# wahn/rs_pbrt

Measured on NVIDIA B200. Metric: Mrays/s, higher is better.
Workload: dtype f32

## Files before the change

### rs_pbrt_b200/csrc/pb_kernels.cuh

```cuda
#pragma once
#include "pb_bsdf.cuh"
#include "pb_interaction.cuh"
#include "pb_sobol.cuh"
#include "pb_texture.cuh"
#include "pb_material.cuh"

namespace pb {

#define PB_TRACE_THREADS 128
#define PB_TRACE_SMEM_BYTES 49152
#define PB_SHADE_THREADS 128
#define PB_SMEM_SOBOL_BYTES 49152

#ifdef PB_HOST_EMU
PB_D void mbar_init(uint64_t*, uint32_t) {}
PB_D void mbar_fence_init() {}
PB_D void mbar_expect_tx(uint64_t*, uint32_t) {}
PB_D void tma_bulk_g2s(void* dst_smem, const void* src_gmem, uint32_t bytes, uint64_t*) { memcpy(dst_smem, src_gmem, bytes); }
PB_D void mbar_wait(uint64_t*, uint32_t) { __syncthreads(); }
#define PB_DYNAMIC_SMEM(name) unsigned char* name = emu::g_dyn_smem
#else
#define PB_DYNAMIC_SMEM(name) extern __shared__ __align__(16) unsigned char name[]
PB_D void mbar_fence_init() { asm volatile("fence.mbarrier_init.release.cluster;" ::: "memory"); }
PB_D uint32_t smem_u32(const void* p) { return (uint32_t)__cvta_generic_to_shared(p); }
// ... 267 lines not shown
    const uint2 a = tris[3 * (size_t)i], b = tris[3 * (size_t)i + 1], c = tris[3 * (size_t)i + 2];
    const uint32_t v0 = a.x, v1 = a.y, v2 = b.x, mesh = b.y, material = c.x;
    const int area_light = (int)c.y;
    uint32_t err = 0;
    if (mesh == 0xffffffffu) {
        if (v0 >= n_instances) err = 5;
        else {
            tv[3 * (size_t)i] = make_float4(__uint_as_float(v0), 0.0f, 0.0f, 0.0f);
            tv[3 * (size_t)i + 1] = make_float4(0.0f, 0.0f, 0.0f, 0.0f);
            tv[3 * (size_t)i + 2] = make_float4(0.0f, __uint_as_float(0xffffffffu), __uint_as_float(0xffffffffu), __uint_as_float((uint32_t)TRI_INSTANCE));
            tidx[i] = make_uint4(0, 0, 0, 0);
        }
    } else if (mesh >= n_meshes) err = 1;
    else {
        const DMeshRec m = meshes[mesh];
        if (v0 >= m.n_verts || v1 >= m.n_verts || v2 >= m.n_verts) err = 2;
        else if (material != 0xffffffffu && material >= n_materials) err = 3;
        else if (area_light >= (int)n_lights) err = 4;
        else if (area_light >= 0 && (m.flags & (TRI_ALPHA | TRI_SHADOW_ALPHA))) err = 6;
        else {
            if (material == 0xffffffffu) status[1] = 1u;
            const float* p0 = vp + 3 * (size_t)(m.vbase + v0);
            const float* p1 = vp + 3 * (size_t)(m.vbase + v1);
            const float* p2 = vp + 3 * (size_t)(m.vbase + v2);
            tv[3 * (size_t)i] = make_float4(p0[0], p0[1], p0[2], p1[0]);
            tv[3 * (size_t)i + 1] = make_float4(p1[1], p1[2], p2[0], p2[1]);
            tv[3 * (size_t)i + 2] = make_float4(p2[2], __uint_as_float(material), __uint_as_float((uint32_t)area_light), __uint_as_float(m.flags));
            tidx[i] = make_uint4(m.vbase + v0, m.vbase + v1, m.vbase + v2, mesh);
        }
    }
    if (err) atomicMax(status, err);
}

__global__ void __launch_bounds__(256) k_wide_build(const float4* __restrict__ nodes, uint32_t n_nodes, float4* __restrict__ wide) {
    const uint32_t i = blockIdx.x * blockDim.x + threadIdx.x;
    if (i >= n_nodes) return;
    const float4 m1 = nodes[2 * (size_t)i + 1];
    const uint32_t meta = __float_as_uint(m1.w);
    if (meta & 0xffffu) return;
    const uint32_t c[2] = {i + 1u, __float_as_uint(m1.z)};
    float4 a[2], b[2];
    uint32_t ref[2];
    for (int k = 0; k < 2; ++k) {
        a[k] = nodes[2 * (size_t)c[k]];
        b[k] = nodes[2 * (size_t)c[k] + 1];
        const uint32_t cm = __float_as_uint(b[k].w), np = cm & 0xffffu;
        ref[k] = np ? (__float_as_uint(b[k].z) | (np << PB_WIDE_LEAF_SHIFT)) : c[k];
    }
    float4* o = wide + 4 * (size_t)i;
    o[0] = make_float4(a[0].x, a[0].y, a[0].z, a[0].w);
    o[1] = make_float4(b[0].x, b[0].y, a[1].x, a[1].y);
    o[2] = make_float4(a[1].z, a[1].w, b[1].x, b[1].y);
    o[3] = make_float4(__uint_as_float(ref[0]), __uint_as_float(ref[1]), __uint_as_float((meta >> 16) & 3u), 0.0f);
}
#ifndef PB_WIDE_MIN_BLOCKS
#define PB_WIDE_MIN_BLOCKS 0
#endif
#ifndef PB_WIDE_INST_MIN_BLOCKS
#define PB_WIDE_INST_MIN_BLOCKS 8
#endif
#if PB_WIDE_MIN_BLOCKS > 0
#define PB_WIDE_BOUNDS __launch_bounds__(PB_TRACE_THREADS, PB_WIDE_MIN_BLOCKS)
#else
#define PB_WIDE_BOUNDS __launch_bounds__(PB_TRACE_THREADS)
#endif
__global__ void PB_WIDE_BOUNDS k_trace_wide_plain(DScene sc, TraceIO io, const uint32_t* __restrict__ d_nrays, uint32_t* __restrict__ cursor, DCounters* cnt, int walk_steps) {
    trace_rays_wide<false>(sc, sc.wide, sc.tri_verts, io, *d_nrays, cursor, cnt, walk_steps);
}
__global__ void __launch_bounds__(PB_TRACE_THREADS, PB_WIDE_INST_MIN_BLOCKS) k_trace_wide_inst(DScene sc, TraceIO io, const uint32_t* __restrict__ d_nrays, uint32_t* __restrict__ cursor,
                                                                                             DCounters* cnt, int walk_steps) {
    trace_rays_wide<true>(sc, sc.wide, sc.tri_verts, io, *d_nrays, cursor, cnt, walk_steps);
}

__global__ void PB_WIDE_BOUNDS k_trace_wide_spec(DScene sc, TraceIO io, const uint32_t* __restrict__ d_nrays,
                                                                                        uint32_t* __restrict__ cursor, DCounters* cnt, int walk_steps) {
    trace_rays_wide_spec(sc, sc.wide, sc.tri_verts, io, *d_nrays, cursor, cnt, walk_steps);
}

__global__ void __launch_bounds__(256) k_rayprep(const float4* __restrict__ rays, const uint32_t* __restrict__ d_nrays, float4* __restrict__ pre) {
    const uint32_t n = *d_nrays;
    for (uint32_t i = blockIdx.x * blockDim.x + threadIdx.x; i < n; i += gridDim.x * blockDim.x) {
        const float4 a = rays[2 * (size_t)i], b = rays[2 * (size_t)i + 1];
        const RayPre r = make_ray(mk3(a.x, a.y, a.z), mk3(b.x, b.y, b.z));
        float4 p0, p1;
        pack_ray(r, p0, p1);
        pre[2 * (size_t)i] = p0;
        pre[2 * (size_t)i + 1] = p1;
    }
}

__global__ void __launch_bounds__(256) k_sort(DScene sc, DPaths ps, DLightGrid grid, uint32_t spatial, uint32_t instancing, const uint32_t* __restrict__ queue,
                                             const uint32_t* __restrict__ d_count, uint32_t* __restrict__ cls_queue, uint32_t cls_stride,
                                             uint32_t* __restrict__ cls_count, uint32_t* __restrict__ reset_count_out, uint32_t* __restrict__ reset_nrays) {
    if (blockIdx.x == 0 && threadIdx.x == 0) { *reset_count_out = 0u; *reset_nrays = 0u; }
    const uint32_t count = *d_count;
    const uint32_t lane = threadIdx.x & 31;
    const uint32_t total = (count + 31u) & ~31u;
    for (uint32_t qi = blockIdx.x * blockDim.x + threadIdx.x; qi < total; qi += gridDim.x * blockDim.x) {
        uint32_t cls = 0xffffffffu, slot = 0;
        if (qi < count) {
            slot = queue[qi];
            cls = 0;
            if (__float_as_uint(ps.L[slot].w) & PF_HAS_RAY) {
                float4 h = ps.hit[slot];
                int prim = __float_as_int(h.x);
                if (prim >= 0) {
                    float4 c = __ldg(sc.tri_verts + 3 * (size_t)prim + 2);
                    uint32_t mat = __float_as_uint(c.y);
                    const uint32_t inst = sc.n_instances ? ps.hit_inst[slot] : 0xffffffffu;
// ... 745 lines not shown
```

### rs_pbrt_b200/csrc/pb_trace.cuh

```cuda
#pragma once
#include "pb_scene.cuh"

namespace pb {

struct RayPre {
    V3 o, d;
    V3 inv_dir;
    int neg[3];
    uint32_t negmask;
    int kx, ky, kz;
    float sx, sy, sz;
};

PB_D RayPre make_ray(V3 o, V3 d) {
    RayPre r;
    r.o = o;
    r.d = d;
    r.inv_dir = mk3(1.0f / d.x, 1.0f / d.y, 1.0f / d.z);
    r.neg[0] = r.inv_dir.x < 0.0f;
    r.neg[1] = r.inv_dir.y < 0.0f;
    r.neg[2] = r.inv_dir.z < 0.0f;
    r.negmask = (uint32_t)r.neg[0] | ((uint32_t)r.neg[1] << 1) | ((uint32_t)r.neg[2] << 2);
    r.kz = maxdim(abs3(d));
    r.kx = r.kz + 1; if (r.kx == 3) r.kx = 0;
// ... 625 lines not shown
            }
            if (!entered) {
                leaf_n = 0;
                if (!done) {
                    uint32_t nxt = 0;
                    PB_WPOP();
                    PB_WGOTO();
                }
            }
        }
        if (active && done) {
            if (INST && !any_hit && !hit_flag) best_prim = -1;
            const uint32_t slot = dest & PB_RAY_SLOT_MASK, kind = dest >> 30;
            if (kind == RAY_SHADOW) io.occl[slot] = best_prim >= 0 ? 1u : 0u;
            else {
                const float4 rec = make_float4(__int_as_float(best_prim), best.b0, best.b1, best.b2);
                if (kind == RAY_EXTEND) { io.hit[slot] = rec; if (INST) io.hit_inst[slot] = (uint32_t)best_inst; }
                else { io.mis_hit[slot] = rec; if (INST) io.mis_inst[slot] = (uint32_t)best_inst; }
            }
            active = false;
        }
    }
#undef PB_WPOP
#undef PB_WGOTO
#undef PB_WPUSH
    uint32_t a = n_closest, b = n_shadow;
    for (int o = 16; o > 0; o >>= 1) { a += __shfl_xor_sync(FULL, a, o); b += __shfl_xor_sync(FULL, b, o); }
    if (lane == 0) {
        if (a) atomicAdd(&cnt->closest_rays, (unsigned long long)a);
        if (b) atomicAdd(&cnt->shadow_rays, (unsigned long long)b);
    }
}

PB_D void trace_rays_wide_spec(const DScene& sc, const float4* __restrict__ wide, const float4* __restrict__ tris, const TraceIO& io, uint32_t n_rays,
                               uint32_t* __restrict__ cursor, DCounters* cnt, int walk_steps) {
    const unsigned FULL = 0xffffffffu;
    const int lane = threadIdx.x & 31;
    constexpr int NS = PB_WIDE_STACK_ENTRIES;
    __shared__ uint32_t s_ref[NS][PB_TRACE_THREADS_];
    __shared__ float s_tmin[NS][PB_TRACE_THREADS_];
    uint32_t l_ref[64 - NS];
    float l_tmin[64 - NS];
    RayPre r;
    float t_max = 0.0f, cur_tmin = 0.0f, leaf2_tmin = 0.0f;
    THit best;
    int best_prim = -1;
    uint32_t sp = 0, cur = 0, dest = 0, leaf1 = 0, leaf2 = 0;
    bool active = false, any_hit = false, exhausted = n_rays == 0, have_cur = false;
    uint32_t n_closest = 0, n_shadow = 0;
    const float neg_inf = __int_as_float((int)0xff800000);
#define PB_SPOP()                                                                                               \
    do {                                                                                                        \
        found = false;                                                                                          \
        while (sp != 0u) {                                                                                      \
            --sp;                                                                                               \
            const uint32_t e_ = sp < (uint32_t)NS ? s_ref[sp][threadIdx.x] : l_ref[sp - NS];                    \
            const float m_ = sp < (uint32_t)NS ? s_tmin[sp][threadIdx.x] : l_tmin[sp - NS];                     \
            if (m_ < t_max) { nxt = e_; tm = m_; found = true; break; }                                         \
        }                                                                                                       \
    } while (0)
#define PB_SROUTE()                                                                                             \
    do {                                                                                                        \
        for (;;) {                                                                                              \
            if (!found) { have_cur = false; break; }                                                            \
            if (!(nxt >> PB_WIDE_LEAF_SHIFT)) { cur = nxt; cur_tmin = tm; have_cur = true; break; }             \
            if (!leaf1) { leaf1 = nxt; PB_SPOP(); continue; }                                                   \
            leaf2 = nxt; leaf2_tmin = tm; have_cur = false; break;                                              \
        }                                                                                                       \
    } while (0)
    for (;;) {
        unsigned idle = __ballot_sync(FULL, !active);
        bool done = false;
        if (idle && !exhausted) {
            uint32_t base = 0;
            if (lane == 0) base = atomicAdd(cursor, (uint32_t)__popc(idle));
            base = __shfl_sync(FULL, base, 0);
            if (base >= n_rays) exhausted = true;
            const uint32_t my = base + (uint32_t)__popc(idle & ((1u << lane) - 1u));
            if (!active && my < n_rays) {
                const uint32_t qi = io.perm ? __ldg(io.perm + my) : my;
                const float4 a = ldg4_stream(io.rays + 2 * (size_t)qi), b = ldg4_stream(io.rays + 2 * (size_t)qi + 1);
                t_max = a.w;
                dest = __float_as_uint(b.w);
                any_hit = (dest >> 30) == RAY_SHADOW;
                r = make_ray(mk3(a.x, a.y, a.z), mk3(b.x, b.y, b.z));
                best_prim = -1;
                best.t = 0.0f; best.b0 = best.b1 = best.b2 = 0.0f;
                sp = 0; cur = 0; cur_tmin = neg_inf; leaf1 = 0; leaf2 = 0;
                active = true;
                if (any_hit) n_shadow++; else n_closest++;
                const float4 n0 = ldg4_keep(sc.nodes), n1 = ldg4_keep(sc.nodes + 1);
                have_cur = slab_test(n0, n1, r, t_max);
            }
        }
        if (!__any_sync(FULL, active)) break;
        for (int step = 0; step < walk_steps; ++step) {
            if (!(active && have_cur)) break;
            const float4* rec = wide + 4 * (size_t)cur;
            const float4 f0 = ldg4_keep(rec), f1 = ldg4_keep(rec + 1), f2 = ldg4_keep(rec + 2), f3 = ldg4_keep(rec + 3);
            float tm0, tm1;
            const bool h0 = slab_geo(f0.x, f0.y, f0.z, f0.w, f1.x, f1.y, r, tm0) && tm0 < t_max;
            const bool h1 = slab_geo(f1.z, f1.w, f2.x, f2.y, f2.z, f2.w, r, tm1) && tm1 < t_max;
            const bool neg = ((r.negmask >> (__float_as_uint(f3.z) & 3u)) & 1u) != 0u;
            const uint32_t ref0 = __float_as_uint(f3.x), ref1 = __float_as_uint(f3.y);
            const uint32_t ref_n = neg ? ref1 : ref0, ref_f = neg ? ref0 : ref1;
            const bool hn = neg ? h1 : h0, hf = neg ? h0 : h1;
            const float tn = neg ? tm1 : tm0, tf = neg ? tm0 : tm1;
            if (hn && hf) {
                if (sp < (uint32_t)NS) { s_ref[sp][threadIdx.x] = ref_f; s_tmin[sp][threadIdx.x] = tf; }
                else { l_ref[sp - NS] = ref_f; l_tmin[sp - NS] = tf; }
                ++sp;
            }
            uint32_t nxt = hn ? ref_n : ref_f;
            float tm = hn ? tn : tf;
            bool found = hn || hf;
            if (!found) PB_SPOP();
            PB_SROUTE();
        }
        if (active && leaf1) {
            const uint32_t leaf_n = leaf1 >> PB_WIDE_LEAF_SHIFT, leaf_off = leaf1 & ((1u << PB_WIDE_LEAF_SHIFT) - 1u);
            for (uint32_t i = 0; i < leaf_n; ++i) {
                const float4* tp = tris + 3 * (size_t)(leaf_off + i);
                const float4 a = ldg4_stream(tp), b = ldg4_stream(tp + 1), c = ldg4_stream(tp + 2);
                THit h;
                if (tri_test(mk3(a.x, a.y, a.z), mk3(a.w, b.x, b.y), mk3(b.z, b.w, c.x), r, t_max, h)) {
                    t_max = h.t;
                    best = h;
                    best_prim = (int)(leaf_off + i);
                    if (any_hit) { done = true; break; }
                }
            }
            leaf1 = 0;
            if (!done) {
                bool resume = false;
                if (leaf2) {
                    if (leaf2_tmin < t_max) leaf1 = leaf2;
                    leaf2 = 0;
                    resume = true;
                } else if (have_cur && !(cur_tmin < t_max)) { have_cur = false; resume = true; }
                if (resume) {
                    uint32_t nxt = 0;
                    float tm = 0.0f;
                    bool found;
                    PB_SPOP();
                    PB_SROUTE();
                }
            }
        }
        if (active && !done && !leaf1 && !leaf2 && !have_cur) done = true;
        if (active && done) {
            const uint32_t slot = dest & PB_RAY_SLOT_MASK, kind = dest >> 30;
            if (kind == RAY_SHADOW) io.occl[slot] = best_prim >= 0 ? 1u : 0u;
            else {
                const float4 rec = make_float4(__int_as_float(best_prim), best.b0, best.b1, best.b2);
                if (kind == RAY_EXTEND) io.hit[slot] = rec; else io.mis_hit[slot] = rec;
            }
            active = false;
        }
    }
#undef PB_SPOP
#undef PB_SROUTE
    uint32_t a = n_closest, b = n_shadow;
    for (int o = 16; o > 0; o >>= 1) { a += __shfl_xor_sync(FULL, a, o); b += __shfl_xor_sync(FULL, b, o); }
    if (lane == 0) {
        if (a) atomicAdd(&cnt->closest_rays, (unsigned long long)a);
        if (b) atomicAdd(&cnt->shadow_rays, (unsigned long long)b);
    }
}

}
```

### rs_pbrt_b200/csrc/pbrt_gpu.cu

```cuda
#include <sched.h>

#include <algorithm>
#include <chrono>
#include <cmath>
#include <cstdio>
#include <cstdlib>
#include <atomic>
#include <cstring>
#include <functional>
#include <map>
#include <memory>
#include <mutex>
#include <string>
#include <thread>
#include <vector>

#include "../../include/pbrt_gpu.h"
#include "pb_kernels.cuh"
#include "pb_direct.cuh"

using namespace pb;

extern "C" {
extern const unsigned char pb_sobol_blob_start[];
// ... 424 lines not shown
    size_t ev_used = 0;
    cudaError_t event(cudaEvent_t* e) {
        if (ev_used == ev_pool.size()) {
            cudaEvent_t n;
            cudaError_t rc = cudaEventCreate(&n);
            if (rc != cudaSuccess) return rc;
            ev_pool.push_back(n);
        }
        *e = ev_pool[ev_used++];
        return cudaSuccess;
    }
    std::mutex mu;
};
static size_t lightgrid_budget() {
    if (const char* e = std::getenv("PB_LIGHTGRID_BYTES")) {
        const long long v = std::atoll(e);
        if (v > 0) return (size_t)v;
    }
    return (size_t)4 << 30;
}
static DeviceScratch* scratch_for(int device) {
    static DeviceScratch* pool[64] = {nullptr};
    static std::mutex pool_mu;
    std::lock_guard<std::mutex> g(pool_mu);
    if (device < 0 || device >= 64) return nullptr;
    if (!pool[device]) pool[device] = new DeviceScratch();
    return pool[device];
}

struct PbrtScene {
    int device = 0;
    DScene d;
    DevBuf<float4> nodes, tri_verts, wide;
    DevBuf<uint4> tri_idx;
    DevBuf<float> vn, vuv, vs;
    DevBuf<DMaterial> materials, materials_single;
    DevBuf<DLight> lights;
    DevBuf<uint32_t> m32, nib;
    DevBuf<uint64_t> vdc, vdci;
    DevBuf<float> halton;
    std::vector<DLight> h_lights;
    std::vector<uint32_t> h_nib;
    struct EnvBufs { DevBuf<float4> texels; DevBuf<float> cond_func, cond_cdf, cond_int, marg_func, marg_cdf; };
    std::vector<std::unique_ptr<EnvBufs>> env_bufs;
    DevBuf<DEnv> envs;
    DevBuf<DInstance> instances;
    DevBuf<uint2> mesh_alpha;
    std::vector<std::unique_ptr<DevBuf<float4>>> tex_bufs;
    DevBuf<DTexture> textures;
    DevBuf<DMatSrc> mat_src;
    DevBuf<float> ewa_lut;
    std::vector<Sp> h_env_power;
    bool has_null_material = false;
    bool area_only = true;
    uint32_t class_mask = 0;
    size_t upload_bytes = 0;
    DevBuf<DCounters> counters;
    DevBuf<float> film, samples;
    size_t capacity = 0;
    void recycle_buffers(int dev) {
        nodes.cache_dev = tri_verts.cache_dev = wide.cache_dev = tri_idx.cache_dev = vn.cache_dev = vuv.cache_dev = vs.cache_dev = dev;
        materials.cache_dev = materials_single.cache_dev = lights.cache_dev = m32.cache_dev = nib.cache_dev = vdc.cache_dev = vdci.cache_dev = halton.cache_dev = dev;
        envs.cache_dev = instances.cache_dev = mesh_alpha.cache_dev = textures.cache_dev = mat_src.cache_dev = ewa_lut.cache_dev = counters.cache_dev = dev;
    }
};

static bool wide_enabled() {
    static const bool on = !(getenv("PB_WIDE") && atoi(getenv("PB_WIDE")) == 0);
    return on;
}
static bool wide_spec_enabled() {
    static const bool on = getenv("PB_WIDE_SPEC") && atoi(getenv("PB_WIDE_SPEC")) != 0;
    return on;
}
struct TraceLauncher {
    bool count_work = false, inst = false, smem = false, alpha = false, wide = false, wide_spec = false;
    int wide_walk = 16;
    size_t smem_bytes = 0;
    int grid = 1, blocks_per_sm = 1;
    template <typename F> void with_kernel(F&& f) const {
        if (alpha) {
            if (inst) { if (count_work) f(k_trace<true, 0, false, true, true>); else f(k_trace<false, 0, false, true, true>); }
            else { if (count_work) f(k_trace<true, 0, false, false, true>); else f(k_trace<false, 0, false, false, true>); }
        } else if (inst) { if (count_work) f(k_trace<true, 0, false, true>); else f(k_trace<false, 0, false, true>); }
        else if (smem) { if (count_work) f(k_trace<true, 0, true>); else f(k_trace<false, 0, true>); }
        else { if (count_work) f(k_trace<true, 0, false>); else f(k_trace<false, 0, false>); }
    }
    cudaError_t init(const PbrtScene* sc, bool count, int sm_count) {
        count_work = count;
        inst = sc->d.n_instances > 0;
        alpha = sc->d.mesh_alpha != nullptr;
        const size_t scene_bytes = (size_t)sc->d.n_nodes * 32 + (size_t)sc->d.n_tris * 48;
        smem = !inst && !alpha && scene_bytes > 0 && scene_bytes <= PB_TRACE_SMEM_BYTES;
        smem_bytes = smem ? scene_bytes : 0;
        wide = wide_enabled() && sc->d.wide != nullptr && !count_work && !alpha && !smem;
        {
            int l2 = 0;
            cudaDeviceGetAttribute(&l2, cudaDevAttrL2CacheSize, sc->device);
            wide_walk = (size_t)sc->d.n_nodes * 64 > (size_t)std::max(l2, 1) ? 6 : 16;
            if (const char* e_ = getenv("PB_WIDE_WALK")) wide_walk = std::min(64, std::max(1, atoi(e_)));
        }
        int bps = 1;
        cudaError_t e = cudaSuccess;
        wide_spec = wide && !inst && wide_spec_enabled();
        if (wide_spec) e = cudaOccupancyMaxActiveBlocksPerMultiprocessor(&bps, k_trace_wide_spec, PB_TRACE_THREADS, 0);
        else if (wide) e = inst ? cudaOccupancyMaxActiveBlocksPerMultiprocessor(&bps, k_trace_wide_inst, PB_TRACE_THREADS, 0)
                           : cudaOccupancyMaxActiveBlocksPerMultiprocessor(&bps, k_trace_wide_plain, PB_TRACE_THREADS, 0);
        else with_kernel([&](auto k) { e = cudaOccupancyMaxActiveBlocksPerMultiprocessor(&bps, k, PB_TRACE_THREADS, smem_bytes); });
        blocks_per_sm = bps;
        grid = sm_count * std::max(1, bps);
        return e;
    }
    void launch(const DScene& d, const TraceIO& io, const uint32_t* d_nrays, uint32_t* d_cursor, DCounters* cnt, cudaStream_t s) const {
        if (wide_spec) k_trace_wide_spec<<<grid, PB_TRACE_THREADS, 0, s>>>(d, io, d_nrays, d_cursor, cnt, wide_walk);
        else if (wide) {
            if (inst) k_trace_wide_inst<<<grid, PB_TRACE_THREADS, 0, s>>>(d, io, d_nrays, d_cursor, cnt, wide_walk);
            else k_trace_wide_plain<<<grid, PB_TRACE_THREADS, 0, s>>>(d, io, d_nrays, d_cursor, cnt, wide_walk);
        } else if (alpha) {
            if (inst) { if (count_work) k_trace<true, 0, false, true, true><<<grid, PB_TRACE_THREADS, 0, s>>>(d, io, d_nrays, 0, d_cursor, cnt); else k_trace<false, 0, false, true, true><<<grid, PB_TRACE_THREADS, 0, s>>>(d, io, d_nrays, 0, d_cursor, cnt); }
            else { if (count_work) k_trace<true, 0, false, false, true><<<grid, PB_TRACE_THREADS, 0, s>>>(d, io, d_nrays, 0, d_cursor, cnt); else k_trace<false, 0, false, false, true><<<grid, PB_TRACE_THREADS, 0, s>>>(d, io, d_nrays, 0, d_cursor, cnt); }
        } else if (inst) {
            if (count_work) k_trace<true, 0, false, true><<<grid, PB_TRACE_THREADS, 0, s>>>(d, io, d_nrays, 0, d_cursor, cnt);
            else k_trace<false, 0, false, true><<<grid, PB_TRACE_THREADS, 0, s>>>(d, io, d_nrays, 0, d_cursor, cnt);
        } else if (smem) {
            if (count_work) k_trace<true, 0, true><<<grid, PB_TRACE_THREADS, smem_bytes, s>>>(d, io, d_nrays, 0, d_cursor, cnt);
            else k_trace<false, 0, true><<<grid, PB_TRACE_THREADS, smem_bytes, s>>>(d, io, d_nrays, 0, d_cursor, cnt);
        } else {
            if (count_work) k_trace<true, 0, false><<<grid, PB_TRACE_THREADS, 0, s>>>(d, io, d_nrays, 0, d_cursor, cnt);
            else k_trace<false, 0, false><<<grid, PB_TRACE_THREADS, 0, s>>>(d, io, d_nrays, 0, d_cursor, cnt);
        }
    }
};

static unsigned host_threads() {
    static const unsigned n = [] {
        unsigned c = std::max(1u, std::thread::hardware_concurrency());
        cpu_set_t set;
        if (sched_getaffinity(0, sizeof set, &set) == 0) c = std::max(1, CPU_COUNT(&set));
        if (FILE* f = fopen("/sys/fs/cgroup/cpu.max", "r")) {
            char quota[32] = {0};
            long period = 0;
            if (fscanf(f, "%31s %ld", quota, &period) == 2 && strcmp(quota, "max") != 0 && period > 0) c = std::min<unsigned>(c, (unsigned)std::max(1L, (atol(quota) + period / 2) / period));
            fclose(f);
        }
        if (const char* w = getenv("LOCAL_WORLD_SIZE")) c = std::max(1u, c / (unsigned)std::max(1, atoi(w)));
        return std::min(32u, c);
    }();
    return n;
// ... 143 lines not shown
        lights[i].kind = l.kind;
        lights[i].L[0] = l.L[0]; lights[i].L[1] = l.L[1]; lights[i].L[2] = l.L[2];
        lights[i].tri = l.tri;
        lights[i].two_sided = l.two_sided ? 1u : 0u;
        for (int k = 0; k < 3; ++k) lights[i].p[k] = l.p[k];
        for (int k = 0; k < 9; ++k) lights[i].w2l[k] = l.w2l[k];
        lights[i].cos_total_width = l.cos_total_width;
        lights[i].cos_falloff_start = l.cos_falloff_start;
        lights[i].area = l.area;
        lights[i].n_samples = l.n_samples ? l.n_samples : 1u;
        if (l.kind == PBRT_LIGHT_INFINITE) {
            const uint32_t w = l.env_res[0], h = l.env_res[1];
            if (!l.env_texels || w == 0 || h == 0) return fail(PBRT_E_INVALID, "infinite light without texels");
            if (w > 16384 || h > 16384) return fail(PBRT_E_UNSUPPORTED, "environment map larger than 16384 texels on a side");
            if (n_inf == PBRT_MAX_INFINITE_LIGHTS) return fail(PBRT_E_UNSUPPORTED, "too many infinite lights");
            inf_idx[n_inf++] = i;
        }
    }
    const unsigned hw = host_threads();
    auto parallel_for = [&](uint32_t n, const std::function<int(uint32_t, uint32_t)>& body) -> int {
        const unsigned nt = n < 65536 ? 1u : hw;
        std::vector<int> rc(nt, 0);
        std::vector<std::thread> th;
        for (unsigned t = 0; t < nt; ++t) {
            uint32_t lo = (uint32_t)((uint64_t)n * t / nt), hi = (uint32_t)((uint64_t)n * (t + 1) / nt);
            if (nt == 1) rc[0] = body(lo, hi);
            else th.emplace_back([&, t, lo, hi] { rc[t] = body(lo, hi); });
        }
        for (auto& x : th) x.join();
        for (int r : rc) if (r) return r;
        return 0;
    };
    static_assert(sizeof(PbrtBvhNode) == 32, "LinearBVHNode layout");
    std::atomic<uint32_t> max_leaf_prims(0);
    int vrc = parallel_for(desc->n_nodes, [&](uint32_t lo, uint32_t hi) -> int {
        uint32_t mx = 0;
        struct Publish { std::atomic<uint32_t>& a; uint32_t& v; ~Publish() { uint32_t c = a.load(); while (v > c && !a.compare_exchange_weak(c, v)) {} } } pub{max_leaf_prims, mx};
        for (uint32_t i = lo; i < hi; ++i) {
            const PbrtBvhNode& n = desc->nodes[i];
            if (n.n_prims > 0) {
                if ((uint64_t)n.offset + n.n_prims > desc->n_tris || n.offset < 0) return 1;
                mx = std::max<uint32_t>(mx, n.n_prims);
            } else if (n.offset <= (int32_t)i || (uint32_t)n.offset >= desc->n_nodes || i + 1 >= desc->n_nodes || n.axis > 2) return 2;
        }
        return 0;
    });
    if (vrc == 1) return fail(PBRT_E_INVALID, "BVH leaf range out of bounds");
    if (vrc == 2) return fail(PBRT_E_INVALID, "BVH interior node malformed");
    since("nodes validated");
    {
        struct Range { uint32_t lo, hi; uint32_t depth; };
        std::vector<Range> work;
        bool layout_ok = true, too_deep = false;
        auto spine_end = [&](uint32_t r) -> uint32_t {
            uint32_t i = r;
            for (;;) {
                const PbrtBvhNode& n = desc->nodes[i];
                if (n.n_prims > 0) return i + 1;
                i = (uint32_t)n.offset;
            }
        };
        if (desc->n_nodes) work.push_back({0u, spine_end(0u), 0u});
        for (uint32_t k = 0; k < desc->n_instances && desc->instances; ++k) {
            const uint32_t r = desc->instances[k].root;
            if (r >= desc->n_nodes) return fail(PBRT_E_INVALID, "instance root out of range");
            bool seen = false;
            for (const Range& w : work) seen |= w.lo == r;
            if (!seen) work.push_back({r, spine_end(r), 0u});
        }
        const uint32_t grain = std::max<uint32_t>(4096u, desc->n_nodes / (8u * hw));
        for (size_t k = 0; k < work.size() && layout_ok && !too_deep;) {
            const Range w = work[k];
            const PbrtBvhNode& n = desc->nodes[w.lo];
            if (w.hi - w.lo <= grain || n.n_prims > 0) { ++k; continue; }
            const uint32_t off = (uint32_t)n.offset;
            if (off <= w.lo + 1 || off >= w.hi) { layout_ok = false; break; }
// ... 229 lines not shown
    std::memcpy(vdc.data(), blob + 32 + m32.size() * 4, vdc.size() * 8);
    std::memcpy(vdci.data(), blob + 32 + m32.size() * 4 + vdc.size() * 8, vdci.size() * 8);
    std::vector<uint32_t> nib((size_t)1024 * PB_SOBOL_CHUNKS * 16);
    for (int dim = 0; dim < 1024; ++dim)
        for (int c = 0; c < PB_SOBOL_CHUNKS; ++c)
            for (int e = 0; e < 16; ++e) {
                uint32_t v = 0;
                for (int j = 0; j < 4; ++j)
                    if (e & (1 << j)) v ^= m32[(size_t)dim * 52 + 4 * c + j];
                nib[((size_t)dim * PB_SOBOL_CHUNKS + c) * 16 + e] = v;
            }
    std::vector<float> halton(128 * 5);
    for (int s = 0; s < 128; ++s)
        for (int k = 0; k < 5; ++k) halton[5 * s + k] = host_radical_inverse(k, (uint64_t)s);

    since("tables built");
    sc->has_null_material = has_null;
    sc->h_nib = nib;
    for (const DLight& l : lights) if (l.kind != PBRT_LIGHT_DIFFUSE_AREA) sc->area_only = false;
    for (const DMaterial& m : mats) sc->class_mask |= 1u << (m.cls & 0xff);
    sc->h_lights = lights;
#define UP(buf, vec)                                                                                     \
    do {                                                                                                 \
        cudaError_t e_ = sc->buf.upload(vec);                                                            \
        if (e_ != cudaSuccess) return fail(PBRT_E_CUDA, std::string("upload " #buf ": ") + cudaGetErrorString(e_)); \
        sc->upload_bytes += (vec).size() * sizeof((vec)[0]);                                             \
    } while (0)
    sc->upload_bytes += up_bytes;
    since("nodes + triangles uploaded");
    {
        bool ok = desc->n_nodes > 1 && desc->nodes[0].n_prims == 0 && !any_alpha &&
                  desc->n_nodes < (1u << PB_WIDE_LEAF_SHIFT) && desc->n_tris < (1u << PB_WIDE_LEAF_SHIFT) &&
                  (desc->n_instances > 0 || (size_t)desc->n_nodes * 32 + (size_t)desc->n_tris * 48 > PB_TRACE_SMEM_BYTES) && max_leaf_prims.load() <= 15u;
        if (ok) {
            CK(sc->wide.alloc(4 * (size_t)desc->n_nodes));
            k_wide_build<<<(desc->n_nodes + 255) / 256, 256>>>(sc->nodes.p, desc->n_nodes, sc->wide.p);
            CK(cudaGetLastError());
            g_launches++;
        }
    }
    {
        std::vector<DEnv> envs;
        sc->h_env_power.assign(desc->n_lights, sp1(0.0f));
        for (uint32_t k = 0; k < n_inf; ++k) {
            const PbrtLight& l = desc->lights[inf_idx[k]];
            HostEnv he;
            build_env(l.env_texels, (int)l.env_res[0], (int)l.env_res[1], he);
            sc->env_bufs.emplace_back(new PbrtScene::EnvBufs());
            PbrtScene::EnvBufs& b = *sc->env_bufs.back();
            cudaError_t e_ = b.texels.upload(he.texels);
            if (e_ == cudaSuccess) e_ = b.cond_func.upload(he.cond_func);
            if (e_ == cudaSuccess) e_ = b.cond_cdf.upload(he.cond_cdf);
            if (e_ == cudaSuccess) e_ = b.cond_int.upload(he.cond_int);
            if (e_ == cudaSuccess) e_ = b.marg_func.upload(he.marg_func);
            if (e_ == cudaSuccess) e_ = b.marg_cdf.upload(he.marg_cdf);
            if (e_ != cudaSuccess) { return fail(PBRT_E_CUDA, std::string("upload environment map: ") + cudaGetErrorString(e_)); }
            sc->upload_bytes += he.texels.size() * 16 + (he.cond_func.size() + he.cond_cdf.size() + he.cond_int.size() + he.marg_func.size() + he.marg_cdf.size()) * 4;
            DEnv de;
            std::memset(&de, 0, sizeof de);
            de.texels = b.texels.p; de.w = he.w; de.h = he.h; de.nu = he.nu; de.nv = he.nv;
            de.cond_func = b.cond_func.p; de.cond_cdf = b.cond_cdf.p; de.cond_int = b.cond_int.p;
            de.marg_func = b.marg_func.p; de.marg_cdf = b.marg_cdf.p; de.marg_int = he.marg_int;
            std::memcpy(de.l2w, l.l2w, sizeof de.l2w);
            std::memcpy(de.w2l, l.w2l, sizeof de.w2l);
            lights[inf_idx[k]].env = (uint32_t)envs.size();
            envs.push_back(de);
            sc->h_env_power[inf_idx[k]] = he.power_L;
        }
        sc->h_lights = lights;
        if (!envs.empty()) UP(envs, envs);
    }
// ... 63 lines not shown
    d.tri_idx = sc->tri_idx.p;
    d.vn = sc->vn.p; d.vuv = sc->vuv.p; d.vs = sc->vs.p;
    d.materials = sc->materials.p; d.n_materials = desc->n_materials;
    d.lights = sc->lights.p; d.n_lights = desc->n_lights;
    d.envs = sc->envs.p; d.n_inf = n_inf;
    d.instances = sc->instances.p; d.n_instances = desc->n_instances;
    d.mesh_alpha = sc->mesh_alpha.p;
    d.textures = sc->textures.p; d.mat_src = sc->mat_src.p; d.ewa_lut = sc->ewa_lut.p; d.n_textures = desc->n_textures;
    {
        auto r2c = [&](float x, float y) {
            const float* m = desc->camera.raster_to_camera;
            V3 r = mk3(m[0] * x + m[1] * y + m[2] * 0.0f + m[3], m[4] * x + m[5] * y + m[6] * 0.0f + m[7], m[8] * x + m[9] * y + m[10] * 0.0f + m[11]);
            const float w = m[12] * x + m[13] * y + m[14] * 0.0f + m[15];
            if (w != 1.0f) { const float inv = 1.0f / w; r = mk3(inv * r.x, inv * r.y, inv * r.z); }
            return r;
        };
        const V3 r0 = r2c(0.0f, 0.0f), dx = r2c(1.0f, 0.0f) - r0, dy = r2c(0.0f, 1.0f) - r0;
        d.dx_camera[0] = dx.x; d.dx_camera[1] = dx.y; d.dx_camera[2] = dx.z;
        d.dy_camera[0] = dy.x; d.dy_camera[1] = dy.y; d.dy_camera[2] = dy.z;
    }
    for (uint32_t k = 0; k < n_inf; ++k) d.inf[k] = inf_idx[k];
    std::memcpy(d.raster_to_camera, desc->camera.raster_to_camera, 64);
    std::memcpy(d.camera_to_world, desc->camera.camera_to_world, 64);
    d.lens_radius = desc->camera.lens_radius; d.focal_distance = desc->camera.focal_distance;
    d.shutter_open = desc->camera.shutter_open; d.shutter_close = desc->camera.shutter_close;
    for (int k = 0; k < 3; ++k) { d.wb_min[k] = desc->world_bound[k]; d.wb_max[k] = desc->world_bound[3 + k]; }
    {
        V3 pmin = mk3(d.wb_min[0], d.wb_min[1], d.wb_min[2]), pmax = mk3(d.wb_max[0], d.wb_max[1], d.wb_max[2]);
        V3 c = vdiv(pmin + pmax, 2.0f);
        bool inside = c.x >= pmin.x && c.x <= pmax.x && c.y >= pmin.y && c.y <= pmax.y && c.z >= pmin.z && c.z <= pmax.z;
        d.world_radius = inside ? len3(c - pmax) : 0.0f;
    }
    CK(cudaDeviceSynchronize());
    stage_lock.unlock();
    *out = sc_guard.release();
    since("done");
    return PBRT_OK;
}

int pbrt_gpu_host_register(const void* ptr, uint64_t bytes) {
    if (!ptr || !bytes) return fail(PBRT_E_INVALID, "null argument");
    cudaError_t e = cudaHostRegister(const_cast<void*>(ptr), (size_t)bytes, cudaHostRegisterPortable);
    if (e != cudaSuccess) { cudaGetLastError(); return fail(PBRT_E_CUDA, std::string("cudaHostRegister: ") + cudaGetErrorString(e)); }
    return PBRT_OK;
}
int pbrt_gpu_host_unregister(const void* ptr) {
    if (!ptr) return fail(PBRT_E_INVALID, "null argument");
    cudaError_t e = cudaHostUnregister(const_cast<void*>(ptr));
    if (e != cudaSuccess) { cudaGetLastError(); return fail(PBRT_E_CUDA, std::string("cudaHostUnregister: ") + cudaGetErrorString(e)); }
    return PBRT_OK;
}

uint64_t pbrt_gpu_scene_bytes(const PbrtScene* scene) { return scene ? (uint64_t)scene->upload_bytes : 0; }

void pbrt_gpu_scene_destroy(PbrtScene* scene) {
    if (!scene) return;
    cudaSetDevice(scene->device);
    delete scene;
}

}

struct Share {
    const int32_t* rect = nullptr;
    uint32_t part = 0, n_parts = 0;
};
// ... 1097 lines not shown
```

Baseline: 2131.

## Compact wide BVH records to interior nodes only for non-instanced scenes

Wide BVH records are now written only for interior nodes in non-instanced scenes. Before, they sat at the original node index, which left leaf-sized holes in the array. A count/scan/rank kernel sequence assigns each interior node a dense index, and child references are remapped to it. The goal is a smaller, denser traversal footprint with better cache-line and L2 use. The walk-step heuristic now uses the compacted record count, which can pick the longer walk on mid-size scenes. The optional speculative trace kernel path (off by default) is removed, and the build gains extra small launches.

Result: no change. 2146 (median of 6 runs) (+0.7%).

```diff
diff --git a/rs_pbrt_b200/csrc/pb_kernels.cuh b/rs_pbrt_b200/csrc/pb_kernels.cuh
--- a/rs_pbrt_b200/csrc/pb_kernels.cuh
+++ b/rs_pbrt_b200/csrc/pb_kernels.cuh
@@ -323,7 +323,51 @@
     if (err) atomicMax(status, err);
 }
 
-__global__ void __launch_bounds__(256) k_wide_build(const float4* __restrict__ nodes, uint32_t n_nodes, float4* __restrict__ wide) {
+__global__ void __launch_bounds__(256) k_wide_count(const float4* __restrict__ nodes, uint32_t n_nodes, uint32_t* __restrict__ block_count) {
+    __shared__ uint32_t s_warp[8];
+    const uint32_t i = blockIdx.x * 256u + threadIdx.x;
+    const bool interior = i < n_nodes && !(__float_as_uint(nodes[2 * (size_t)i + 1].w) & 0xffffu);
+    const unsigned m = __ballot_sync(0xffffffffu, interior);
+    if ((threadIdx.x & 31) == 0) s_warp[threadIdx.x >> 5] = (uint32_t)__popc(m);
+    __syncthreads();
+    if (threadIdx.x == 0) {
+        uint32_t t = 0;
+        for (int w = 0; w < 8; ++w) t += s_warp[w];
+        block_count[blockIdx.x] = t;
+    }
+}
+__global__ void __launch_bounds__(1024) k_wide_scan(uint32_t* __restrict__ c, uint32_t n) {
+    __shared__ uint32_t s_run[1024];
+    const uint32_t per = (n + 1023u) / 1024u;
+    const uint32_t lo = threadIdx.x * per < n ? threadIdx.x * per : n, hi = lo + per < n ? lo + per : n;
+    uint32_t t = 0;
+    for (uint32_t k = lo; k < hi; ++k) t += c[k];
+    s_run[threadIdx.x] = t;
+    __syncthreads();
+    if (threadIdx.x == 0) {
+        uint32_t run = 0;
+        for (int k = 0; k < 1024; ++k) { const uint32_t v = s_run[k]; s_run[k] = run; run += v; }
+    }
+    __syncthreads();
+    uint32_t run = s_run[threadIdx.x];
+    for (uint32_t k = lo; k < hi; ++k) { const uint32_t v = c[k]; c[k] = run; run += v; }
+}
+__global__ void __launch_bounds__(256) k_wide_rank(const float4* __restrict__ nodes, uint32_t n_nodes, const uint32_t* __restrict__ block_first,
+                                                   uint32_t* __restrict__ rank) {
+    __shared__ uint32_t s_warp[8];
+    const uint32_t i = blockIdx.x * 256u + threadIdx.x;
+    const int lane = threadIdx.x & 31, warp = threadIdx.x >> 5;
+    const bool interior = i < n_nodes && !(__float_as_uint(nodes[2 * (size_t)i + 1].w) & 0xffffu);
+    const unsigned m = __ballot_sync(0xffffffffu, interior);
+    if (lane == 0) s_warp[warp] = (uint32_t)__popc(m);
+    __syncthreads();
+    uint32_t before = block_first[blockIdx.x];
+    for (int w = 0; w < warp; ++w) before += s_warp[w];
+    if (interior) rank[i] = before + (uint32_t)__popc(m & ((1u << lane) - 1u));
+}
+
+__global__ void __launch_bounds__(256) k_wide_build(const float4* __restrict__ nodes, uint32_t n_nodes, const uint32_t* __restrict__ rank,
+                                                    float4* __restrict__ wide) {
     const uint32_t i = blockIdx.x * blockDim.x + threadIdx.x;
     if (i >= n_nodes) return;
     const float4 m1 = nodes[2 * (size_t)i + 1];
@@ -336,9 +380,9 @@
         a[k] = nodes[2 * (size_t)c[k]];
         b[k] = nodes[2 * (size_t)c[k] + 1];
         const uint32_t cm = __float_as_uint(b[k].w), np = cm & 0xffffu;
-        ref[k] = np ? (__float_as_uint(b[k].z) | (np << PB_WIDE_LEAF_SHIFT)) : c[k];
-    }
-    float4* o = wide + 4 * (size_t)i;
+        ref[k] = np ? (__float_as_uint(b[k].z) | (np << PB_WIDE_LEAF_SHIFT)) : rank ? rank[c[k]] : c[k];
+    }
+    float4* o = wide + 4 * (size_t)(rank ? rank[i] : i);
     o[0] = make_float4(a[0].x, a[0].y, a[0].z, a[0].w);
     o[1] = make_float4(b[0].x, b[0].y, a[1].x, a[1].y);
     o[2] = make_float4(a[1].z, a[1].w, b[1].x, b[1].y);
@@ -361,11 +405,6 @@
 __global__ void __launch_bounds__(PB_TRACE_THREADS, PB_WIDE_INST_MIN_BLOCKS) k_trace_wide_inst(DScene sc, TraceIO io, const uint32_t* __restrict__ d_nrays, uint32_t* __restrict__ cursor,
                                                                                              DCounters* cnt, int walk_steps) {
     trace_rays_wide<true>(sc, sc.wide, sc.tri_verts, io, *d_nrays, cursor, cnt, walk_steps);
-}
-
-__global__ void PB_WIDE_BOUNDS k_trace_wide_spec(DScene sc, TraceIO io, const uint32_t* __restrict__ d_nrays,
-                                                                                        uint32_t* __restrict__ cursor, DCounters* cnt, int walk_steps) {
-    trace_rays_wide_spec(sc, sc.wide, sc.tri_verts, io, *d_nrays, cursor, cnt, walk_steps);
 }
 
 __global__ void __launch_bounds__(256) k_rayprep(const float4* __restrict__ rays, const uint32_t* __restrict__ d_nrays, float4* __restrict__ pre) {
diff --git a/rs_pbrt_b200/csrc/pb_trace.cuh b/rs_pbrt_b200/csrc/pb_trace.cuh
--- a/rs_pbrt_b200/csrc/pb_trace.cuh
+++ b/rs_pbrt_b200/csrc/pb_trace.cuh
@@ -681,140 +681,4 @@
     }
 }
 
-PB_D void trace_rays_wide_spec(const DScene& sc, const float4* __restrict__ wide, const float4* __restrict__ tris, const TraceIO& io, uint32_t n_rays,
-                               uint32_t* __restrict__ cursor, DCounters* cnt, int walk_steps) {
-    const unsigned FULL = 0xffffffffu;
-    const int lane = threadIdx.x & 31;
-    constexpr int NS = PB_WIDE_STACK_ENTRIES;
-    __shared__ uint32_t s_ref[NS][PB_TRACE_THREADS_];
-    __shared__ float s_tmin[NS][PB_TRACE_THREADS_];
-    uint32_t l_ref[64 - NS];
-    float l_tmin[64 - NS];
-    RayPre r;
-    float t_max = 0.0f, cur_tmin = 0.0f, leaf2_tmin = 0.0f;
-    THit best;
-    int best_prim = -1;
-    uint32_t sp = 0, cur = 0, dest = 0, leaf1 = 0, leaf2 = 0;
-    bool active = false, any_hit = false, exhausted = n_rays == 0, have_cur = false;
-    uint32_t n_closest = 0, n_shadow = 0;
-    const float neg_inf = __int_as_float((int)0xff800000);
-#define PB_SPOP()                                                                                               \
-    do {                                                                                                        \
-        found = false;                                                                                          \
-        while (sp != 0u) {                                                                                      \
-            --sp;                                                                                               \
-            const uint32_t e_ = sp < (uint32_t)NS ? s_ref[sp][threadIdx.x] : l_ref[sp - NS];                    \
-            const float m_ = sp < (uint32_t)NS ? s_tmin[sp][threadIdx.x] : l_tmin[sp - NS];                     \
-            if (m_ < t_max) { nxt = e_; tm = m_; found = true; break; }                                         \
-        }                                                                                                       \
-    } while (0)
-#define PB_SROUTE()                                                                                             \
-    do {                                                                                                        \
-        for (;;) {                                                                                              \
-            if (!found) { have_cur = false; break; }                                                            \
-            if (!(nxt >> PB_WIDE_LEAF_SHIFT)) { cur = nxt; cur_tmin = tm; have_cur = true; break; }             \
-            if (!leaf1) { leaf1 = nxt; PB_SPOP(); continue; }                                                   \
-            leaf2 = nxt; leaf2_tmin = tm; have_cur = false; break;                                              \
-        }                                                                                                       \
-    } while (0)
-    for (;;) {
-        unsigned idle = __ballot_sync(FULL, !active);
-        bool done = false;
-        if (idle && !exhausted) {
-            uint32_t base = 0;
-            if (lane == 0) base = atomicAdd(cursor, (uint32_t)__popc(idle));
-            base = __shfl_sync(FULL, base, 0);
-            if (base >= n_rays) exhausted = true;
-            const uint32_t my = base + (uint32_t)__popc(idle & ((1u << lane) - 1u));
-            if (!active && my < n_rays) {
-                const uint32_t qi = io.perm ? __ldg(io.perm + my) : my;
-                const float4 a = ldg4_stream(io.rays + 2 * (size_t)qi), b = ldg4_stream(io.rays + 2 * (size_t)qi + 1);
-                t_max = a.w;
-                dest = __float_as_uint(b.w);
-                any_hit = (dest >> 30) == RAY_SHADOW;
-                r = make_ray(mk3(a.x, a.y, a.z), mk3(b.x, b.y, b.z));
-                best_prim = -1;
-                best.t = 0.0f; best.b0 = best.b1 = best.b2 = 0.0f;
-                sp = 0; cur = 0; cur_tmin = neg_inf; leaf1 = 0; leaf2 = 0;
-                active = true;
-                if (any_hit) n_shadow++; else n_closest++;
-                const float4 n0 = ldg4_keep(sc.nodes), n1 = ldg4_keep(sc.nodes + 1);
-                have_cur = slab_test(n0, n1, r, t_max);
-            }
-        }
-        if (!__any_sync(FULL, active)) break;
-        for (int step = 0; step < walk_steps; ++step) {
-            if (!(active && have_cur)) break;
-            const float4* rec = wide + 4 * (size_t)cur;
-            const float4 f0 = ldg4_keep(rec), f1 = ldg4_keep(rec + 1), f2 = ldg4_keep(rec + 2), f3 = ldg4_keep(rec + 3);
-            float tm0, tm1;
-            const bool h0 = slab_geo(f0.x, f0.y, f0.z, f0.w, f1.x, f1.y, r, tm0) && tm0 < t_max;
-            const bool h1 = slab_geo(f1.z, f1.w, f2.x, f2.y, f2.z, f2.w, r, tm1) && tm1 < t_max;
-            const bool neg = ((r.negmask >> (__float_as_uint(f3.z) & 3u)) & 1u) != 0u;
-            const uint32_t ref0 = __float_as_uint(f3.x), ref1 = __float_as_uint(f3.y);
-            const uint32_t ref_n = neg ? ref1 : ref0, ref_f = neg ? ref0 : ref1;
-            const bool hn = neg ? h1 : h0, hf = neg ? h0 : h1;
-            const float tn = neg ? tm1 : tm0, tf = neg ? tm0 : tm1;
-            if (hn && hf) {
-                if (sp < (uint32_t)NS) { s_ref[sp][threadIdx.x] = ref_f; s_tmin[sp][threadIdx.x] = tf; }
-                else { l_ref[sp - NS] = ref_f; l_tmin[sp - NS] = tf; }
-                ++sp;
-            }
-            uint32_t nxt = hn ? ref_n : ref_f;
-            float tm = hn ? tn : tf;
-            bool found = hn || hf;
-            if (!found) PB_SPOP();
-            PB_SROUTE();
-        }
-        if (active && leaf1) {
-            const uint32_t leaf_n = leaf1 >> PB_WIDE_LEAF_SHIFT, leaf_off = leaf1 & ((1u << PB_WIDE_LEAF_SHIFT) - 1u);
-            for (uint32_t i = 0; i < leaf_n; ++i) {
-                const float4* tp = tris + 3 * (size_t)(leaf_off + i);
-                const float4 a = ldg4_stream(tp), b = ldg4_stream(tp + 1), c = ldg4_stream(tp + 2);
-                THit h;
-                if (tri_test(mk3(a.x, a.y, a.z), mk3(a.w, b.x, b.y), mk3(b.z, b.w, c.x), r, t_max, h)) {
-                    t_max = h.t;
-                    best = h;
-                    best_prim = (int)(leaf_off + i);
-                    if (any_hit) { done = true; break; }
-                }
-            }
-            leaf1 = 0;
-            if (!done) {
-                bool resume = false;
-                if (leaf2) {
-                    if (leaf2_tmin < t_max) leaf1 = leaf2;
-                    leaf2 = 0;
-                    resume = true;
-                } else if (have_cur && !(cur_tmin < t_max)) { have_cur = false; resume = true; }
-                if (resume) {
-                    uint32_t nxt = 0;
-                    float tm = 0.0f;
-                    bool found;
-                    PB_SPOP();
-                    PB_SROUTE();
-                }
-            }
-        }
-        if (active && !done && !leaf1 && !leaf2 && !have_cur) done = true;
-        if (active && done) {
-            const uint32_t slot = dest & PB_RAY_SLOT_MASK, kind = dest >> 30;
-            if (kind == RAY_SHADOW) io.occl[slot] = best_prim >= 0 ? 1u : 0u;
-            else {
-                const float4 rec = make_float4(__int_as_float(best_prim), best.b0, best.b1, best.b2);
-                if (kind == RAY_EXTEND) io.hit[slot] = rec; else io.mis_hit[slot] = rec;
-            }
-            active = false;
-        }
-    }
-#undef PB_SPOP
-#undef PB_SROUTE
-    uint32_t a = n_closest, b = n_shadow;
-    for (int o = 16; o > 0; o >>= 1) { a += __shfl_xor_sync(FULL, a, o); b += __shfl_xor_sync(FULL, b, o); }
-    if (lane == 0) {
-        if (a) atomicAdd(&cnt->closest_rays, (unsigned long long)a);
-        if (b) atomicAdd(&cnt->shadow_rays, (unsigned long long)b);
-    }
-}
-
-}
+}
diff --git a/rs_pbrt_b200/csrc/pbrt_gpu.cu b/rs_pbrt_b200/csrc/pbrt_gpu.cu
--- a/rs_pbrt_b200/csrc/pbrt_gpu.cu
+++ b/rs_pbrt_b200/csrc/pbrt_gpu.cu
@@ -480,6 +480,8 @@
     int device = 0;
     DScene d;
     DevBuf<float4> nodes, tri_verts, wide;
+    DevBuf<uint32_t> wide_rank;
+    uint32_t n_wide_records = 0;
     DevBuf<uint4> tri_idx;
     DevBuf<float> vn, vuv, vs;
     DevBuf<DMaterial> materials, materials_single;
@@ -507,7 +509,7 @@
     DevBuf<float> film, samples;
     size_t capacity = 0;
     void recycle_buffers(int dev) {
-        nodes.cache_dev = tri_verts.cache_dev = wide.cache_dev = tri_idx.cache_dev = vn.cache_dev = vuv.cache_dev = vs.cache_dev = dev;
+        nodes.cache_dev = tri_verts.cache_dev = wide.cache_dev = wide_rank.cache_dev = tri_idx.cache_dev = vn.cache_dev = vuv.cache_dev = vs.cache_dev = dev;
         materials.cache_dev = materials_single.cache_dev = lights.cache_dev = m32.cache_dev = nib.cache_dev = vdc.cache_dev = vdci.cache_dev = halton.cache_dev = dev;
         envs.cache_dev = instances.cache_dev = mesh_alpha.cache_dev = textures.cache_dev = mat_src.cache_dev = ewa_lut.cache_dev = counters.cache_dev = dev;
     }
@@ -517,12 +519,8 @@
     static const bool on = !(getenv("PB_WIDE") && atoi(getenv("PB_WIDE")) == 0);
     return on;
 }
-static bool wide_spec_enabled() {
-    static const bool on = getenv("PB_WIDE_SPEC") && atoi(getenv("PB_WIDE_SPEC")) != 0;
-    return on;
-}
 struct TraceLauncher {
-    bool count_work = false, inst = false, smem = false, alpha = false, wide = false, wide_spec = false;
+    bool count_work = false, inst = false, smem = false, alpha = false, wide = false;
     int wide_walk = 16;
     size_t smem_bytes = 0;
     int grid = 1, blocks_per_sm = 1;
@@ -545,14 +543,12 @@
         {
             int l2 = 0;
             cudaDeviceGetAttribute(&l2, cudaDevAttrL2CacheSize, sc->device);
-            wide_walk = (size_t)sc->d.n_nodes * 64 > (size_t)std::max(l2, 1) ? 6 : 16;
+            wide_walk = (size_t)sc->n_wide_records * 64 > (size_t)std::max(l2, 1) ? 6 : 16;
             if (const char* e_ = getenv("PB_WIDE_WALK")) wide_walk = std::min(64, std::max(1, atoi(e_)));
         }
         int bps = 1;
         cudaError_t e = cudaSuccess;
-        wide_spec = wide && !inst && wide_spec_enabled();
-        if (wide_spec) e = cudaOccupancyMaxActiveBlocksPerMultiprocessor(&bps, k_trace_wide_spec, PB_TRACE_THREADS, 0);
-        else if (wide) e = inst ? cudaOccupancyMaxActiveBlocksPerMultiprocessor(&bps, k_trace_wide_inst, PB_TRACE_THREADS, 0)
+        if (wide) e = inst ? cudaOccupancyMaxActiveBlocksPerMultiprocessor(&bps, k_trace_wide_inst, PB_TRACE_THREADS, 0)
                            : cudaOccupancyMaxActiveBlocksPerMultiprocessor(&bps, k_trace_wide_plain, PB_TRACE_THREADS, 0);
         else with_kernel([&](auto k) { e = cudaOccupancyMaxActiveBlocksPerMultiprocessor(&bps, k, PB_TRACE_THREADS, smem_bytes); });
         blocks_per_sm = bps;
@@ -560,8 +556,7 @@
         return e;
     }
     void launch(const DScene& d, const TraceIO& io, const uint32_t* d_nrays, uint32_t* d_cursor, DCounters* cnt, cudaStream_t s) const {
-        if (wide_spec) k_trace_wide_spec<<<grid, PB_TRACE_THREADS, 0, s>>>(d, io, d_nrays, d_cursor, cnt, wide_walk);
-        else if (wide) {
+        if (wide) {
             if (inst) k_trace_wide_inst<<<grid, PB_TRACE_THREADS, 0, s>>>(d, io, d_nrays, d_cursor, cnt, wide_walk);
             else k_trace_wide_plain<<<grid, PB_TRACE_THREADS, 0, s>>>(d, io, d_nrays, d_cursor, cnt, wide_walk);
         } else if (alpha) {
@@ -771,16 +766,20 @@
         return 0;
     };
     static_assert(sizeof(PbrtBvhNode) == 32, "LinearBVHNode layout");
-    std::atomic<uint32_t> max_leaf_prims(0);
+    std::atomic<uint32_t> max_leaf_prims(0), n_interior(0);
     int vrc = parallel_for(desc->n_nodes, [&](uint32_t lo, uint32_t hi) -> int {
-        uint32_t mx = 0;
+        uint32_t mx = 0, ni = 0;
         struct Publish { std::atomic<uint32_t>& a; uint32_t& v; ~Publish() { uint32_t c = a.load(); while (v > c && !a.compare_exchange_weak(c, v)) {} } } pub{max_leaf_prims, mx};
+        struct Count { std::atomic<uint32_t>& a; uint32_t& v; ~Count() { a += v; } } cnt{n_interior, ni};
         for (uint32_t i = lo; i < hi; ++i) {
             const PbrtBvhNode& n = desc->nodes[i];
             if (n.n_prims > 0) {
                 if ((uint64_t)n.offset + n.n_prims > desc->n_tris || n.offset < 0) return 1;
                 mx = std::max<uint32_t>(mx, n.n_prims);
-            } else if (n.offset <= (int32_t)i || (uint32_t)n.offset >= desc->n_nodes || i + 1 >= desc->n_nodes || n.axis > 2) return 2;
+            } else {
+                if (n.offset <= (int32_t)i || (uint32_t)n.offset >= desc->n_nodes || i + 1 >= desc->n_nodes || n.axis > 2) return 2;
+                ++ni;
+            }
         }
         return 0;
     });
@@ -1076,11 +1075,24 @@
         bool ok = desc->n_nodes > 1 && desc->nodes[0].n_prims == 0 && !any_alpha &&
                   desc->n_nodes < (1u << PB_WIDE_LEAF_SHIFT) && desc->n_tris < (1u << PB_WIDE_LEAF_SHIFT) &&
                   (desc->n_instances > 0 || (size_t)desc->n_nodes * 32 + (size_t)desc->n_tris * 48 > PB_TRACE_SMEM_BYTES) && max_leaf_prims.load() <= 15u;
-        if (ok) {
+        if (ok && desc->n_instances > 0) {
             CK(sc->wide.alloc(4 * (size_t)desc->n_nodes));
-            k_wide_build<<<(desc->n_nodes + 255) / 256, 256>>>(sc->nodes.p, desc->n_nodes, sc->wide.p);
+            k_wide_build<<<(desc->n_nodes + 255) / 256, 256>>>(sc->nodes.p, desc->n_nodes, nullptr, sc->wide.p);
             CK(cudaGetLastError());
             g_launches++;
+            sc->n_wide_records = desc->n_nodes;
+        } else if (ok) {
+            const uint32_t nb = (desc->n_nodes + 255u) / 256u;
+            CK(sc->wide_rank.alloc((size_t)desc->n_nodes + nb));
+            CK(sc->wide.alloc(4 * (size_t)n_interior.load()));
+            uint32_t* counts = sc->wide_rank.p + desc->n_nodes;
+            k_wide_count<<<nb, 256>>>(sc->nodes.p, desc->n_nodes, counts);
+            k_wide_scan<<<1, 1024>>>(counts, nb);
+            k_wide_rank<<<nb, 256>>>(sc->nodes.p, desc->n_nodes, counts, sc->wide_rank.p);
+            k_wide_build<<<nb, 256>>>(sc->nodes.p, desc->n_nodes, sc->wide_rank.p, sc->wide.p);
+            CK(cudaGetLastError());
+            g_launches += 4;
+            sc->n_wide_records = n_interior.load();
         }
     }
     {
@@ -1210,6 +1222,7 @@
         d.world_radius = inside ? len3(c - pmax) : 0.0f;
     }
     CK(cudaDeviceSynchronize());
+    sc->wide_rank.release();
     stage_lock.unlock();
     *out = sc_guard.release();
     since("done");
```
